# IanMadlenya/pyconsensus

Hardware: AMD Instinct MI355X
Metric: oracle rounds/sec (batched 50x20, 1 GPU) (higher is better)
Workload: dtype f64; 1 GPU; C3: 65536 independent 50x20 oracle rounds per GPU per step (one wavefront per round), inputs resident in HBM, every output of the result dict written (original and filled included); rounds_per_gpu=65536, reporters=50, events=20, parallelism=rounds sharded across 1 GPU(s), no collective

## Files before the change

pyconsensus_amd/csrc/pcx_api.cpp:

```cpp
#include <hip/hip_runtime.h>

#include <algorithm>
#include <atomic>
#include <cstdio>
#include <cstdlib>
#include <new>
#include <string>
#include <thread>
#include <vector>

#include "../../include/pcx.h"
#include "pcx_host.h"
#include "pcx_internal.h"
#include "pcx_seqsum.h"
#include "pcx_sync.h"

namespace pcx {
namespace host __attribute__((visibility("hidden"))) {
thread_local std::string g_err;

int fail(int code, const std::string& msg) {
    g_err = msg;
    return code;
}

int hip_fail(hipError_t e, const char* what) {
    return fail(PCX_EHIP, std::string(what) + ": " + hipGetErrorString(e));
}

void stamps_begin(pcx::BatchArgs& a, hipStream_t stream) {
    const char* env = getenv("PCX_STAMPS");
    if (!env || env[0] != '1' || a.B <= 0) return;
    const size_t bytes = (size_t)a.B * 32 * sizeof(long long);
    long long* d = nullptr;
    if (hipMalloc(&d, bytes) != hipSuccess) return;
    (void)hipMemsetAsync(d, 0, bytes, stream);
    a.stamps = d;
}

std::vector<long long> stamps_end(pcx::BatchArgs& a, hipStream_t stream) {
    std::vector<long long> h(a.stamps ? a.B * 32 : 0);
    if (!a.stamps) return h;
    (void)hipMemcpyAsync(h.data(), a.stamps, h.size() * sizeof(long long), hipMemcpyDeviceToHost, stream);
    (void)hipStreamSynchronize(stream);
    (void)hipFree(a.stamps);
    a.stamps = nullptr;
    return h;
}

int medium_scratch_reserve(pcx_ctx* ctx, size_t need) {
    if (ctx->mscr_bytes >= need) return PCX_OK;
    if (ctx->mscr) (void)hipFree(ctx->mscr);
    ctx->mscr = nullptr;
    ctx->mscr_bytes = 0;
    const hipError_t e = hipMalloc(&ctx->mscr, need);
    if (e != hipSuccess) return hip_fail(e, "hipMalloc(medium scratch)");
    ctx->mscr_bytes = need;
    return PCX_OK;
}
}
}
using namespace pcx::host;

extern "C" {

int pcx_abi_version(void) { return PCX_ABI_VERSION; }

const char* pcx_last_error(void) { return g_err.c_str(); }

namespace {
pcx_ctx* new_ctx(int device_id, const char* who) {
    int n = 0;
    hipError_t e = hipGetDeviceCount(&n);
    if (e != hipSuccess || device_id < 0 || device_id >= n) {
        g_err = std::string(who) + ": no HIP device " + std::to_string(device_id);
        return nullptr;
    }
    pcx_ctx* c = new (std::nothrow) pcx_ctx;
    if (!c) {
        g_err = std::string(who) + ": out of host memory";
        return nullptr;
    }
    c->device = device_id;
    return c;
}

pcx_ctx* with_comm(pcx_ctx* c, pcx::Comm* comm, const std::string& err) {
    if (!c) return nullptr;
    if (!comm) {
        g_err = err.empty() ? "communicator setup failed" : err;
        delete c;
        return nullptr;
    }
    c->comm = comm;
    return c;
}
}

pcx_ctx* pcx_create(int device_id) { return new_ctx(device_id, "pcx_create"); }

int pcx_comm_unique_id(pcx_comm_id* out) {
    if (!out) return fail(PCX_EINVAL, "pcx_comm_unique_id: null argument");
    std::string err;
    const int rc = pcx::comm_rccl_unique_id(out, err);
    return rc ? fail(rc, err) : PCX_OK;
}

pcx_ctx* pcx_create_rank(int device_id, int world, int rank, const pcx_comm_id* id) {
    if (!id || world < 1 || rank < 0 || rank >= world) {
        g_err = "pcx_create_rank: bad id / world / rank";
        return nullptr;
    }
    pcx_ctx* c = new_ctx(device_id, "pcx_create_rank");
    if (!c) return nullptr;
    std::string err;
    return with_comm(c, pcx::comm_rccl(device_id, world, rank, id, err), err);
}

pcx_group* pcx_group_create(int world) {
    pcx_group* g = pcx::group_create(world);
    if (!g) g_err = "pcx_group_create: world must be >= 1";
    return g;
}

void pcx_group_destroy(pcx_group* g) { pcx::group_destroy(g); }

pcx_ctx* pcx_create_grouped(int device_id, pcx_group* g, int rank) {
    pcx_ctx* c = new_ctx(device_id, "pcx_create_grouped");
    if (!c) return nullptr;
    std::string err;
    return with_comm(c, pcx::comm_group(g, rank, err), err);
}

pcx_ctx* pcx_create_custom(int device_id, int world, int rank, const pcx_comm_ops* ops) {
    pcx_ctx* c = new_ctx(device_id, "pcx_create_custom");
    if (!c) return nullptr;
    std::string err;
    return with_comm(c, pcx::comm_custom(world, rank, ops, err), err);
}

pcx_ctx* pcx_create_devices(int n_devices, const int* device_ids) {
    if (n_devices < 1 || !device_ids) {
        g_err = "pcx_create_devices: need n_devices >= 1 and device_ids";
        return nullptr;
    }
    pcx_ctx* c = new_ctx(device_ids[0], "pcx_create_devices");
    if (!c) return nullptr;
    for (int k = 1; k < n_devices; k++) {
        pcx_ctx* probe = new_ctx(device_ids[k], "pcx_create_devices");
        if (!probe) {
            delete c;
            return nullptr;
        }
        delete probe;
    }
    bool distinct = true;
    for (int a = 0; a < n_devices; a++)
        for (int b = a + 1; b < n_devices; b++) distinct = distinct && device_ids[a] != device_ids[b];
    std::string err;
    std::vector<pcx::Comm*> comms;
    if (distinct) {
        const int rc = pcx::comm_rccl_all(n_devices, device_ids, comms, err);
        if (rc) {
            g_err = "pcx_create_devices: " + err;
            delete c;
            return nullptr;
        }
    } else {
        c->group = pcx::group_create(n_devices);
        for (int k = 0; k < n_devices && c->group; k++) comms.push_back(pcx::comm_group(c->group, k, err));
    }
    for (int k = 0; k < n_devices; k++) {
        pcx_ctx* s = (k < (int)comms.size() && comms[k]) ? new (std::nothrow) pcx_ctx : nullptr;
        if (s) {
            s->device = device_ids[k];
            s->comm = comms[k];
        } else if (k < (int)comms.size()) {
            delete comms[k];
        }
        c->sub.push_back(s);
    }
    for (pcx_ctx* s : c->sub)
        if (!s) {
            g_err = "pcx_create_devices: communicator setup failed" + (err.empty() ? std::string() : ": " + err);
            pcx_destroy(c);
            return nullptr;
        }
    return c;
}

int pcx_ctx_world(const pcx_ctx* ctx) {
    if (ctx && !ctx->sub.empty()) return (int)ctx->sub.size();
    return ctx && ctx->comm ? ctx->comm->world : 1;
}
int pcx_ctx_rank(const pcx_ctx* ctx) { return ctx && ctx->comm ? ctx->comm->rank : 0; }

int pcx_ctx_usable(const pcx_ctx* ctx) {
    if (!ctx) return 0;
    if (ctx->comm && ctx->comm->aborted) return 0;
    for (const pcx_ctx* s : ctx->sub)
        if (s->comm && s->comm->aborted) return 0;
    return 1;
}

int pcx_release_workspace(pcx_ctx* ctx) {
    if (!ctx) return fail(PCX_EINVAL, "pcx_release_workspace: null context");
    for (pcx_ctx* s : ctx->sub) pcx_release_workspace(s);
    pcx::rounds_free(ctx);
    (void)hipSetDevice(ctx->device);
    pcx::workspace_free(ctx);
    pcx::io_bufs_free(ctx);
    pcx::sim_free(ctx);
    pcx::ragged_free(ctx);
    return PCX_OK;
}

}
namespace pcx {
void ctx_host_free(pcx_ctx* c) {
    if (c->mscr) (void)hipFree(c->mscr);
    c->mscr = nullptr;
    c->mscr_bytes = 0;
    if (c->pinned) (void)hipHostFree(c->pinned);
    c->pinned = nullptr;
    c->pinned_bytes = 0;
    if (c->sel_pin) (void)hipHostFree(c->sel_pin);
    c->sel_pin = nullptr;
    if (c->pin_small) (void)hipHostFree(c->pin_small);
    c->pin_small = nullptr;
    c->pin_small_bytes = 0;
    for (hipEvent_t& ev : c->sel_ev) {
        if (ev) (void)hipEventDestroy(ev);
        ev = nullptr;
    }
    if (c->side_stream) (void)hipStreamDestroy(c->side_stream);
    c->side_stream = nullptr;
    io_bufs_free(c);
}
void sim_free(pcx_ctx* c) {
    if (c->sim_buf) (void)hipFree(c->sim_buf);
    c->sim_buf = nullptr;
    c->sim_bytes = 0;
}
void ragged_free(pcx_ctx* c) {
    for (auto& s : c->rag) {
        if (s.copy_ev) (void)hipEventSynchronize(s.copy_ev);
        if (s.kern_ev) (void)hipEventSynchronize(s.kern_ev);
        if (s.pin) (void)hipHostFree(s.pin);
        if (s.dev) (void)hipFree(s.dev);
        if (s.copy_ev) (void)hipEventDestroy(s.copy_ev);
        if (s.kern_ev) (void)hipEventDestroy(s.kern_ev);
        s = pcx_ctx::RaggedSlot();
    }
}
void io_bufs_free(pcx_ctx* c) {
    for (auto& b : c->io_bufs)
        if (b.first) (void)hipFree(b.first);
    c->io_bufs.clear();
}
}
extern "C" {

void pcx_destroy(pcx_ctx* ctx) {
    if (!ctx) return;
    for (pcx_ctx* s : ctx->sub) pcx_destroy(s);
    if (ctx->group) pcx::group_destroy(ctx->group);
    pcx::rounds_free(ctx);
    (void)hipSetDevice(ctx->device);
    pcx::ctx_host_free(ctx);
    pcx::workspace_free(ctx);
    pcx::sim_free(ctx);
    pcx::ragged_free(ctx);
    delete ctx->comm;
    delete ctx;
}

int pcx_set_stream(pcx_ctx* ctx, void* s) {
    if (!ctx) return fail(PCX_EINVAL, "pcx_set_stream: null context");
    ctx->stream = reinterpret_cast<hipStream_t>(s);
    return PCX_OK;
}

int pcx_synchronize(pcx_ctx* ctx) {
    if (!ctx) return fail(PCX_EINVAL, "pcx_synchronize: null context");
    hipError_t e = hipSetDevice(ctx->device);
    if (e == hipSuccess) e = hipStreamSynchronize(ctx->stream);
    return e == hipSuccess ? PCX_OK : hip_fail(e, "pcx_synchronize");
}

static int batched_route(int64_t N, int64_t E, int alg, int k) {
    if (N < 1 || N > 0x7fffffff || E < 1 || E > 65536 || alg < PCX_ALG_PCA || alg > PCX_ALG_CLUSTERFECK) return -1;
    const bool large = N > 64 || E > 32;
    if (alg == PCX_ALG_KMEANS && (k < 1 || k > (large ? 1024 : 8) || k > N)) return -1;
    if (!large) return PCX_ROUTE_WAVE;
    return pcx::medium_fits((int)N, (int)E, alg, k) ? PCX_ROUTE_WORKGROUP : PCX_ROUTE_SCHEDULER;
}

int pcx_batched_route(int n_reporters, int n_events, int algorithm, int kmeans_k) {
    return batched_route(n_reporters, n_events, algorithm, kmeans_k);
}

static void print_wave_stamps(const std::vector<long long>& h, int64_t B) {
    static const int order[] = {0, 1, 2, 13, 14, 3, 4, 5, 6, 7, 8, 15, 16, 9, 10, 11, 12};
    const int no = (int)(sizeof(order) / sizeof(order[0]));
    double acc[32] = {0};
    for (int64_t b = 0; b < B; b++)
        for (int k = 1; k < no; k++) {
            const long long t1 = h[b * 32 + order[k]], t0 = h[b * 32 + order[k - 1]];
            if (t1 && t0) acc[order[k]] += (double)(t1 - t0);
        }
    fprintf(stderr, "PCX_STAMPS mean cycles per phase:");
    for (int k = 1; k < no; k++) fprintf(stderr, " %d:%.0f", order[k], acc[order[k]] / (double)B);
    double sort = 0, walk = 0, fast = 0, slow = 0;
    for (int64_t b = 0; b < B; b++) {
        sort += (double)h[b * 32 + 20];
        walk += (double)h[b * 32 + 21];
        fast += (double)h[b * 32 + 22];
        slow += (double)h[b * 32 + 23];
    }
    double iscr = 0, isort = 0;
    for (int64_t b = 0; b < B; b++) {
        iscr += (double)h[b * 32 + 24];
        isort += (double)h[b * 32 + 25];
    }
    fprintf(stderr, " median_sort:%.0f median_walk:%.0f outcome_shortcut:%.4f outcome_sorted:%.4f", sort / (double)B,
            walk / (double)B, fast / (double)B, slow / (double)B);
    fprintf(stderr, " interp_screened:%.4f interp_sorted:%.4f\n", iscr / (double)B, isort / (double)B);
}

static void print_medium_stamps(const std::vector<long long>& h, int64_t B) {
    double acc[16] = {0};
    for (int64_t b = 0; b < B; b++)
        for (int k = 1, prev = 0; k < 16; k++) {
            const long long t1 = h[b * 32 + k], t0 = h[b * 32 + prev];
            if (t1 && t0) {
                acc[k] += (double)(t1 - t0);
                prev = k;
            }
        }
    fprintf(stderr, "PCX_STAMPS medium mean cycles per phase:");
    for (int k = 1; k < 16; k++) fprintf(stderr, " %d:%.0f", k, acc[k] / (double)B);
    double mp[3] = {0, 0, 0};
    for (int64_t b = 0; b < B; b++)
        for (int k = 0; k < 3; k++) mp[k] += (double)h[b * 32 + 20 + k];
    fprintf(stderr, " wave0 medians total:%.0f rank:%.0f walk:%.0f", mp[0] / (double)B, mp[1] / (double)B,
            mp[2] / (double)B);
    double sub[4] = {0, 0, 0, 0};
    for (int64_t b = 0; b < B; b++)
        for (int k = 0; k < 4; k++) {
            const long long t1 = h[b * 32 + 24 + k], t0 = h[b * 32 + (k ? 23 + k : 8)];
            if (t1 && t0) sub[k] += (double)(t1 - t0);
        }
    fprintf(stderr, " nc: minmax+norm:%.0f n12:%.0f dots:%.0f ranks:%.0f", sub[0] / (double)B, sub[1] / (double)B,
            sub[2] / (double)B, sub[3] / (double)B);
    double pw[2] = {0, 0};
    for (int64_t b = 0; b < B; b++) {
        const long long* hb = &h[b * 32];
        if (hb[28] && hb[6]) pw[0] += (double)(hb[28] - hb[6]);
        if (hb[29] && hb[28]) pw[1] += (double)(hb[29] - hb[28]);
    }
    fprintf(stderr, " pi: presq:%.0f steps:%.0f\n", pw[0] / (double)B, pw[1] / (double)B);
}

static int run_workgroup_route(pcx_ctx* ctx, pcx::BatchArgs& a) {
    const int64_t chunk = pcx::medium_chunk(a, MEDIUM_SCRATCH_CAP);
    if (const int rc = medium_scratch_reserve(ctx, pcx::medium_scratch_per_round(a) * (size_t)chunk)) return rc;
    hipError_t e = hipSuccess;
    double* Fscr = (double*)ctx->mscr;
    double* Cscr = Fscr + (a.filled ? 0 : (size_t)chunk * a.N * a.E);
    double* Xscr = Cscr + (size_t)chunk * a.E * a.E;
    stamps_begin(a, ctx->stream);
    for (int64_t b0 = 0; b0 < a.B && e == hipSuccess; b0 += chunk)
        e = pcx::launch_medium(a, b0, std::min<int64_t>(chunk, a.B - b0), Fscr, Cscr, Xscr, ctx->stream);
    if (a.stamps) print_medium_stamps(stamps_end(a, ctx->stream), a.B);
    return e == hipSuccess ? PCX_OK : hip_fail(e, "medium_round_kernel launch");
}

int pcx_consensus_batched_f64(pcx_ctx* ctx, const pcx_batch* in, pcx_batch_result* out) {
    if (!ctx || !in || !out) return fail(PCX_EINVAL, "pcx_consensus_batched_f64: null argument");
    if (in->n_rounds < 0 || in->n_rounds > 0x7fffffff)
        return fail(PCX_EINVAL, "batched: n_rounds must be in [0, 2^31)");
    if (in->n_reporters < 1 || in->n_reporters > 0x7fffffff)
        return fail(PCX_EINVAL, "batched: n_reporters must be in [1, 2^31)");
    if (in->n_events < 1 || in->n_events > 65536) return fail(PCX_EINVAL, "batched: n_events must be in [1, 65536]");
    const bool large = in->n_reporters > 64 || in->n_events > 32;
    const char* own = nullptr;
    if (in->algorithm < PCX_ALG_PCA || in->algorithm > PCX_ALG_CLUSTERFECK)
        own = "algorithm must be an enum pcx_algorithm value (0..7)";
    else if (in->algorithm == PCX_ALG_KMEANS &&
             (!in->kmeans_init || in->kmeans_k < 1 || in->kmeans_k > (large ? 1024 : 8) ||
              in->kmeans_k > in->n_reporters || in->kmeans_restarts < 1))
        own = "k-means needs kmeans_init and 1 <= kmeans_k <= min(N, 8; 1024 above 64 x 32), restarts >= 1";
    else if (in->algorithm == PCX_ALG_BIG_FIVE && (in->max_components < 1 || in->max_components > in->n_events))
        own = "big-five needs 1 <= max_components <= n_events";
    if (const int rc = check_options("batched", in, own)) return rc;
    hipError_t e = hipSetDevice(ctx->device);
    if (e != hipSuccess) return hip_fail(e, "hipSetDevice");
    pcx::BatchArgs a = shared_args(in, out);
    a.B = in->n_rounds;
    a.N = (int)in->n_reporters;
    a.E = (int)in->n_events;
    a.ES = a.E | 1;
    a.bounds_shared = in->bounds_shared;
    a.kmeans_k = in->kmeans_k;
    a.kmeans_restarts = in->kmeans_restarts;
    a.kmeans_init = in->kmeans_init;
    const int route = batched_route(in->n_reporters, in->n_events, in->algorithm, in->kmeans_k);
    if (route < 0) return fail(PCX_EINVAL, "batched: invalid shape or algorithm");
    if (route == PCX_ROUTE_WORKGROUP && !getenv("PCX_NO_MEDIUM")) return run_workgroup_route(ctx, a);
    if (route != PCX_ROUTE_WAVE) {
        std::string err;
        const int rc = pcx::run_rounds(ctx, in, out, err);
        return rc ? fail(rc, "pcx_consensus_batched_f64: " + err) : PCX_OK;
    }
    stamps_begin(a, ctx->stream);
    e = pcx::launch_batched(a, ctx->stream);
    if (a.stamps) print_wave_stamps(stamps_end(a, ctx->stream), a.B);
    return e == hipSuccess ? PCX_OK : hip_fail(e, "batched_round_kernel launch");
}

namespace {
int run_devices(pcx_ctx* ctx, const pcx_problem* p, pcx_result* r, int entry, const double* scores, int rank_rule,
                double* nc, std::string& err) {
    const int n = (int)ctx->sub.size();
    const int64_t N = p->n_rows, E = p->n_events;
    if (p->mem_kind != PCX_MEM_HOST) {
        err = "a multi-device context takes the matrix in host memory (PCX_MEM_HOST)";
        return PCX_EINVAL;
    }
    if (p->n_total != N || p->row_offset != 0) {
        err = "a multi-device context takes the whole matrix (n_total == n_rows, row_offset 0)";
        return PCX_EINVAL;
    }
    if (N < n || E < 1 || !p->reports) {
        err = "bad shape (fewer rows than devices) or missing reports";
        return PCX_EINVAL;
    }
    if (const int rc = pcx::check_problem(p, n, entry, err)) return rc;
    std::vector<pcx_problem> ps(n, *p);
    std::vector<pcx_result> rs(n);
    std::vector<std::string> errs(n);
    std::vector<int> rcs;
    const int64_t base = N / n, rem = N % n;
    auto at = [](double* a, int64_t off) { return a ? a + off : nullptr; };
    for (int k = 0; k < n; k++) {
        const int64_t off = k * base + (k < rem ? k : rem), cnt = base + (k < rem ? 1 : 0);
        pcx_problem& q = ps[k];
        q.n_rows = cnt;
        q.n_total = N;
        q.row_offset = off;
        q.reports = p->reports + off * E;
        q.aux_scores = p->aux_scores ? p->aux_scores + off : nullptr;
        pcx_result& o = rs[k];
        o = pcx_result{};
        o.old_rep = at(r->old_rep, off);
        o.this_rep = at(r->this_rep, off);
        o.smooth_rep = at(r->smooth_rep, off);
        o.scores = at(r->scores, off);
        o.na_row = at(r->na_row, off);
        o.participation_rows = at(r->participation_rows, off);
        o.relative_part = at(r->relative_part, off);
        o.reporter_bonus = at(r->reporter_bonus, off);
        o.original = at(r->original, off * E);
        o.filled = at(r->filled, off * E);
        if (k == 0) {
            o.adj_first_loadings = r->adj_first_loadings;
            o.outcomes_raw = r->outcomes_raw;
            o.outcomes_adjusted = r->outcomes_adjusted;
            o.outcomes_final = r->outcomes_final;
            o.certainty = r->certainty;
            o.consensus_reward = r->consensus_reward;
            o.nas_filled = r->nas_filled;
            o.participation_columns = r->participation_columns;
            o.author_bonus = r->author_bonus;
            o.weighted_mean = r->weighted_mean;
            o.covariance = r->covariance;
        }
    }
    pcx::run_workers(
        n,
        [&](int k) {
            const int64_t off = ps[k].row_offset;
            return pcx::run_matrix(ctx->sub[k], &ps[k], &rs[k], entry, scores ? scores + off : nullptr, rank_rule,
                                   nc ? nc + off : nullptr, errs[k]);
        },
        [&](int k) {
            if (ctx->group) pcx::group_abort(ctx->group);
            for (pcx_ctx* o : ctx->sub)
                if (o->comm && o != ctx->sub[k]) o->comm->abort();
        },
        rcs);
    if (ctx->group) pcx::group_reset(ctx->group);
    int first = -1;
    for (int k = 0; k < n && first < 0; k++)
        if (rcs[k] && errs[k].find("exchange aborted") == std::string::npos) first = k;
    for (int k = first < 0 ? 0 : first; k < n; k++)
        if (rcs[k]) {
            err = "device " + std::to_string(ctx->sub[k]->device) + " (rank " + std::to_string(k) + "): " + errs[k];
            return rcs[k];
        }
    double bytes = 0;
    for (int k = 0; k < n; k++) bytes += rs[k].comm_bytes;
    const pcx_result& z = rs[0];
    r->participation = z.participation;
    r->avg_certainty = z.avg_certainty;
    r->branch = z.branch;
    r->flags = z.flags;
    r->pi_iters = z.pi_iters;
    r->components = z.components;
    r->n_hard = z.n_hard;
    r->sel_passes = z.sel_passes;
    r->comm_bytes = bytes;
    r->grid_events = z.grid_events;
    r->mixed_int8 = z.mixed_int8;
    return 0;
}

int run(pcx_ctx* ctx, const pcx_problem* p, pcx_result* r, int entry, const double* scores, int rank_rule, double* nc,
        const char* who) {
    if (!ctx || !p || !r) return fail(PCX_EINVAL, std::string(who) + ": null argument");
    std::string err;
    if (!ctx->sub.empty()) {
        const int rc = run_devices(ctx, p, r, entry, scores, rank_rule, nc, err);
        return rc ? fail(rc, std::string(who) + ": " + err) : PCX_OK;
    }
    const int rc = pcx::run_matrix(ctx, p, r, entry, scores, rank_rule, nc, err);
    return rc ? fail(rc, std::string(who) + ": " + err) : PCX_OK;
}
}

int pcx_consensus_f64(pcx_ctx* ctx, const pcx_problem* p, pcx_result* r) {
    return run(ctx, p, r, 0, nullptr, 0, nullptr, "pcx_consensus_f64");
}

int pcx_interpolate_f64(pcx_ctx* ctx, const pcx_problem* p, pcx_result* r) {
    return run(ctx, p, r, 1, nullptr, 0, nullptr, "pcx_interpolate_f64");
}

int pcx_wpca_f64(pcx_ctx* ctx, const pcx_problem* p, pcx_result* r) {
    return run(ctx, p, r, 2, nullptr, 0, nullptr, "pcx_wpca_f64");
}

int pcx_lie_detector_f64(pcx_ctx* ctx, const pcx_problem* p, pcx_result* r) {
    return run(ctx, p, r, 3, nullptr, 0, nullptr, "pcx_lie_detector_f64");
}

int pcx_nonconformity_f64(pcx_ctx* ctx, const pcx_problem* p, const double* scores, int rank_rule, double* nc,
                          pcx_result* r) {
    if (!scores || !nc) return fail(PCX_EINVAL, "pcx_nonconformity_f64: scores and nc are required");
    return run(ctx, p, r, 4, scores, rank_rule, nc, "pcx_nonconformity_f64");
}

int pcx_profile_enable(pcx_ctx* ctx, int on) {
    if (!ctx) return fail(PCX_EINVAL, "pcx_profile_enable: null context");
    for (pcx_ctx* s : ctx->sub) s->profile = on ? 1 : 0;
    ctx->profile = on ? 1 : 0;
    return PCX_OK;
}

int pcx_profile_read(pcx_ctx* ctx, double* ms) {
    if (!ctx || !ms) return fail(PCX_EINVAL, "pcx_profile_read: null argument");
    const pcx_ctx* src = ctx->sub.empty() ? ctx : ctx->sub[0];
    for (int k = 0; k < PCX_NSTAGES; k++) ms[k] = src->stage_ms[k];
    return PCX_OK;
}

const char* pcx_stage_name(int k) { return pcx::stage_name(k); }

int pcx_ctx_progress(const pcx_ctx* ctx, int* stage, int* host_waiting) {
    if (!ctx || !stage || !host_waiting) return fail(PCX_EINVAL, "pcx_ctx_progress: null argument");
    const pcx_ctx* src = ctx->sub.empty() ? ctx : ctx->sub[0];
    *stage = src->progress_stage.load(std::memory_order_relaxed);
    *host_waiting = src->progress_wait.load(std::memory_order_relaxed);
    return PCX_OK;
}

double pcx_seqsum_const(double c, int64_t k) { return pcx::seqsum_const(c, k); }

int64_t pcx_seqsum_first_above(double c, double t, int64_t kmax) { return pcx::seqsum_first_above(c, t, kmax); }
int pcx_mixed_digits(void) { return PCX_NDIG; }
int pcx_rccl_version(int* runtime, int* compiled) { return pcx::rccl_version(runtime, compiled); }
int pcx_selftest_abort_once(int users, int aborters, int iters) {
    return pcx::selftest_abort_once(users, aborters, iters, 0);
}
int pcx_selftest_abort_slow_holder(int users, int aborters) {
    return pcx::selftest_abort_once(users, aborters, 1, 1);
}
int pcx_selftest_group_abort(int world, int steps, int fail_rank, int fail_step) {
    return pcx::selftest_group_abort(world, steps, fail_rank, fail_step);
}
int pcx_selftest_rounds_sched(int workers, int64_t rounds, int enomem_worker, int64_t fail_round) {
    return pcx::selftest_rounds_sched(workers, rounds, enomem_worker, fail_round);
}
int pcx_selftest_chunked_copy(int64_t bytes, int64_t chunk, int slots, int threads, int64_t fail_chunk) {
    return pcx::selftest_chunked_copy(bytes, chunk, slots, threads, fail_chunk);
}
int64_t pcx_medium_lds_bytes(int n_reporters, int n_events, int algorithm) {
    if (!pcx::medium_fits(n_reporters, n_events, algorithm, 1)) return 0;
    return (int64_t)pcx::medium_lds_bytes(n_reporters, n_events, algorithm);
}

int64_t pcx_batched_lds_bytes(int n_reporters, int n_events, int algorithm) {
    if (n_reporters < 1 || n_reporters > 64 || n_events < 1 || n_events > 32) return -1;
    return (int64_t)pcx::batched_lds_bytes(n_reporters, n_events, algorithm);
}
int pcx_test_inject_enomem(pcx_ctx* ctx, int worker) {
    if (!ctx) return fail(PCX_EINVAL, "pcx_test_inject_enomem: null context");
    ctx->test_enomem_worker = worker;
    return PCX_OK;
}

}
```

pyconsensus_amd/csrc/pcx_batched_round.inc:

```
#if PCX_ROUND_RAGGED >= 2
#define PCX_ROUND_CELL0 rcell
#define PCX_ROUND_ROW0 rrow
#define PCX_ROUND_EV0 rev
#define PCX_ROUND_B rround
template <int NT, int ET, bool CLUS, bool PK>
#if PCX_ROUND_RAGGED == 3
__global__ void __launch_bounds__(64, 3) ragged_kmeans_round_kernel(BatchArgs ka, const MediumDesc* __restrict__ rag,
                                                                    const RoundParams* __restrict__ ptab,
                                                                    const KmeansEntry* __restrict__ ktab) {
#else
__global__ void __launch_bounds__(64, 3) ragged_params_round_kernel(BatchArgs ka, const MediumDesc* __restrict__ rag,
                                                                    const RoundParams* __restrict__ ptab) {
#endif
    static_assert(NT == 0 && ET == 0, "a ragged launch has no compiled shape");
    extern __shared__ __attribute__((aligned(16))) double smem[];
    const MediumDesc* const rd = rag + blockIdx.x;
    const int N = __builtin_amdgcn_readfirstlane(rd->N), E = __builtin_amdgcn_readfirstlane(rd->E), ES = E | 1;
    const int64_t rcell = uniform64(rd->cell), rrow = uniform64(rd->row), rev = uniform64(rd->ev);
    const int64_t rround = __builtin_amdgcn_readfirstlane(rd->round);
    const RoundParams* const rp = ptab + __builtin_amdgcn_readfirstlane(rd->param);
    BatchArgs a = ka;
    a.algorithm = __builtin_amdgcn_readfirstlane(rp->algorithm);
    a.max_components = __builtin_amdgcn_readfirstlane(rp->max_components);
    a.catch_tol = uniform_f64(rp->catch_tol);
    a.alpha = uniform_f64(rp->alpha);
    a.variance_threshold = uniform_f64(rp->variance_threshold);
    a.hierarchy_threshold = uniform_f64(rp->hierarchy_threshold);
    a.cluster_threshold = uniform_f64(rp->cluster_threshold);
#if PCX_ROUND_RAGGED == 3
    const KmeansEntry* const ke = ktab + rround;
    a.kmeans_k = __builtin_amdgcn_readfirstlane(ke->k);
    a.kmeans_init = ka.kmeans_init + uniform64(ke->offset);
#endif
#elif PCX_ROUND_RAGGED
#define PCX_ROUND_CELL0 rcell
#define PCX_ROUND_ROW0 rrow
#define PCX_ROUND_EV0 rev
#define PCX_ROUND_B blockIdx.x
template <int NT, int ET, bool CLUS, bool PK>
__global__ void __launch_bounds__(64, 3) ragged_round_kernel(BatchArgs a, const RaggedDesc* __restrict__ rag) {
    static_assert(NT == 0 && ET == 0, "a ragged launch has no compiled shape");
    extern __shared__ __attribute__((aligned(16))) double smem[];
    const RaggedDesc* const rd = rag + blockIdx.x;
    const int N = __builtin_amdgcn_readfirstlane(rd->N), E = __builtin_amdgcn_readfirstlane(rd->E), ES = E | 1;
    const int64_t rcell = uniform64(rd->cell), rrow = uniform64(rd->row), rev = uniform64(rd->ev);
#else
#define PCX_ROUND_CELL0 (b * (int64_t)N * E)
#define PCX_ROUND_ROW0 (b * N)
#define PCX_ROUND_EV0 (b * E)
#define PCX_ROUND_B blockIdx.x
template <int NT, int ET, bool CLUS, bool PK>
__global__ void __launch_bounds__(64, (NT > 0 && PK) ? PACKED_WAVES : 3) batched_round_kernel(BatchArgs a) {
    extern __shared__ __attribute__((aligned(16))) double smem[];
    const int N = NT > 0 ? NT : a.N, E = ET > 0 ? ET : a.E, ES = ET > 0 ? compiled_es(ET) : a.ES;
#endif
    const int l = lane_id();
    const int64_t b = PCX_ROUND_B;
    constexpr int NRM = NT > 0 ? NT : 64;
    Smem S = carve(smem, N, E, ES, NRM, PK);
    const bool row = l < N, col = l < E;
    const int64_t bo = a.bounds_shared ? 0 : PCX_ROUND_EV0;
    const bool has_bounds = a.scaled != nullptr;
    auto pw_rows = [&](double v) { return wave_pw_sum_prefix<NT>(v, N); };
    auto pw_cols = [&](double v) { return wave_pw_sum_prefix<ET>(v, E); };
    constexpr int CR = live_rows(ET);

    typedef const __attribute__((address_space(4))) BatchArgs* KernArgs;
    auto out_args = [&]() -> KernArgs {
        uint64_t p = (uint64_t)__builtin_amdgcn_kernarg_segment_ptr();
        asm volatile("" : "+s"(p));
        return (KernArgs)p;
    };

    long long mprof[3] = {0, 0, 0};
    STAMP(0);
    const double* Rg = a.reports + PCX_ROUND_CELL0;
    bool scj = false;
    double loj = 0.0, hij = 0.0;
    if (col && has_bounds) {
        scj = a.scaled[bo + l] != 0;
        loj = a.lo[bo + l];
        hij = a.hi[bo + l];
    }
    double raw = row && a.reputation ? a.reputation[PCX_ROUND_ROW0 + l] : 0.0;
    if constexpr (NT > 0 && ET > 0 && (NT * ET) % 2 == 0) {
        constexpr int TOT2 = NT * ET / 2, NV = (TOT2 + W - 1) / W;
        double2 v[NV];
#pragma unroll
        for (int q = 0; q < NV; q++)
            if (l + W * q < TOT2) v[q] = reinterpret_cast<const double2*>(Rg)[l + W * q];
#pragma unroll
        for (int q = 0; q < NV; q++) {
            const int idx = 2 * (l + W * q);
            if (idx < NT * ET) {
                const int i0 = idx / ET, j0 = idx - i0 * ET;
                const int i1 = (idx + 1) / ET, j1 = idx + 1 - i1 * ET;
                S.F[i0 * ES + j0] = v[q].x;
                S.F[i1 * ES + j1] = v[q].y;
            }
        }
    } else {
        for (int idx = l; idx < N * E; idx += W) {
            const int i = idx / E, j = idx - i * E;
            S.F[i * ES + j] = Rg[idx];
        }
    }
    const uint64_t scaled_mask = ballot(col && scj);

    double rep;
    if (a.reputation) {
        const double tot = pw_rows(raw);
        rep = raw / tot;
    } else {
        rep = 1.0 / (double)N;
    }
    const double tok = trunc(rep * 1e6);
    if (row) S.rep[l] = rep;
    const double denom = tree_sum(row ? tok : 0.0) - 1.0;
    wsync();

    STAMP(1);
    uint32_t nacnt = 0;
    double xnext = row ? S.F[l * ES] : 1.0;
    uint32_t nanb = 0, zerob = 0;
    int zcol = 0;
#pragma unroll(ET > 0 ? ET : 1)
    for (int j = 0; j < E; j++) {
        const bool sc = (scaled_mask >> j) & 1;
        double x = xnext;
        if (j + 1 < E) xnext = row ? S.F[l * ES + j + 1] : 1.0;
        if (sc) {
            const double lo = bcast(loj, j), hi = bcast(hij, j);
            if (row) {
                x = (x - lo) / (hi - lo);
                if (a.int_dtype) x = trunc(x);
                S.F[l * ES + j] = x;
            }
        }
        const bool xn = __builtin_isnan(x), xz = x == 0.0;
        nanb |= xn ? 1u << j : 0u;
        zerob |= xz ? 1u << j : 0u;
        const uint64_t zm = ballot(xz), mm = ballot(xn) | zm;
        zcol = l == j ? popc(zm) : zcol;
        if (l == 0) S.miss[j] = mm;
        asm volatile("" : "+v"(nanb), "+v"(zerob), "+v"(zcol));
    }
    nacnt = (uint32_t)__popc(zerob) | ((uint32_t)__popc(nanb) << 8) | ((uint32_t)zcol << 16);
    wsync();
    if (double* const og = out_args()->original) round_to_global(og + PCX_ROUND_CELL0, S.F, N, E, ES, NT, ET);

    STAMP(2);
    uint64_t miss_j = 0;
    if (col) miss_j = S.miss[l];
    {
        constexpr int NR = NT > 0 ? NT : 64;
        double tot = 0.0, sp = 0.0, sa = 0.0;
#pragma unroll 10
        for (int i = 0; i < NR; i++) {
            if (i < N) {
                const bool miss = (miss_j >> i) & 1;
                const double re = miss ? 0.0 : S.rep[i];
                const double f = miss ? 0.0 : S.F[i * ES + (col ? l : 0)];
                tot = tot + re;
                sp = fma(re, f, sp);
                sa = fma(fabs(re), fabs(f), sa);
            }
        }
        const double t_lo = 1.5 - a.catch_tol, t_hi = 1.5 + a.catch_tol;
        const double accf = sp / tot, margin = 1e-12 * (sa / tot);
        const bool binary_fill = col && miss_j && !scj;
        const bool fast = tot > 0.0 && __builtin_isfinite(accf) && __builtin_isfinite(margin) &&
                          fabs(accf - t_lo) > margin && fabs(accf - t_hi) > margin;
        double acc = accf;
        if (ballot(binary_fill && !fast)) {
            double ex = 0.0;
#pragma unroll
            for (int i = 0; i < NR; i++) {
                if (i < N) {
                    const double t = (S.rep[i] / tot) * S.F[i * ES + (col ? l : 0)];
                    ex = ((miss_j >> i) & 1) ? ex : ex + t;
                }
            }
            if (!fast) acc = ex;
        }
        if (binary_fill) {
            double g = catch_(acc, a.catch_tol);
            if (a.int_dtype) g = trunc(g);
            S.guess[l] = g;
        }
        if (col && miss_j) S.tot[l] = tot;
    }
    wsync();
    STAMP(13);
    {
        uint64_t todo = ballot(col && scj && miss_j != 0);
        auto pair_of = [&](int j, double& x, double& w, bool& present) {
            const uint64_t mj = S.miss[j];
            present = row && !((mj >> l) & 1);
            const double tot = S.tot[j];
            x = row ? S.F[l * ES + j] : 0.0;
            w = present ? S.rep[l] / tot : 0.0;
        };
        auto finish = [&](int j, double g) {
            if (a.int_dtype) g = trunc(g);
            if (l == 0) S.guess[j] = g;
        };
        constexpr int NRS = NT > 0 ? NT : 64, KP = (NRS + 3) & ~3;
        const uint64_t all_j = todo;
        if (todo && a.reputation && !ballot(row && !(rep >= 0.0))) {
            uint32_t* const kx = reinterpret_cast<uint32_t*>(S.M);
            float* const wf = reinterpret_cast<float*>(S.M) + KP;
            if (l < KP) wf[l] = row ? (float)rep : 0.f;
            for (uint64_t t = todo; t; t &= t - 1) {
                const int j = __builtin_ctzll(t);
                const uint64_t mj = S.miss[j];
                const bool present = row && !((mj >> l) & 1);
                const double x0 = row ? S.F[l * ES + j] : 0.0;
                double g;
                if (wave_wmedian_screen<NRS>(x0, rep, present, S.tot[j], N, kx, wf, g)) {
                    finish(j, g);
                    todo &= ~(1ull << j);
                }
            }
            wsync();
        }
        if (a.stamps && l == 0) {
            a.stamps[b * 32 + 24] = popc(all_j) - popc(todo);
            a.stamps[b * 32 + 25] = popc(todo);
        }
        while (todo) {
            const int j = __builtin_ctzll(todo);
            todo &= todo - 1;
            double x0, w0;
            bool p0;
            pair_of(j, x0, w0, p0);
            finish(j, wave_wmedian_rank<(NT > 0 ? NT : 64)>(x0, w0, p0, N, S.M, a.stamps ? mprof : nullptr));
            wsync();
        }
    }
    wsync();
    STAMP(14);
    if (row) {
        uint64_t mn = S.miss[0];
        double gn = S.guess[0];
        for (int j = 0; j < E; j++) {
            const uint64_t mj = mn;
            const double g = gn;
            if (j + 1 < E) {
                mn = S.miss[j + 1];
                gn = S.guess[j + 1];
            }
            if ((mj >> l) & 1) S.F[l * ES + j] = g;
        }
    }
    wsync();
    if (double* const fg = out_args()->filled) round_to_global(fg + PCX_ROUND_CELL0, S.F, N, E, ES, NT, ET);

    STAMP(3);
    double oldj = col ? ob_vecmat(S.rep, S.F + l, ES, N, E, l) : 0.0;

    double sc_i = 0.0, nc_i = 0.0, ld_j = 0.0;
    int branch = 5, flags = 0, iters = 0, comps = -1;
    const int alg = a.algorithm;
    const bool clus = CLUS && alg >= 5;
    const double rep_sum = pw_rows(rep);
    if (alg == 0 || alg == 2 || alg == 3 || clus) {
        const double den = rep_sum;
        double muj = 0.0;
        if (E == 1) {
            const double p = row ? S.F[l * ES] * rep : 0.0;
            const double acc = pw_rows(p);
            muj = acc / den;
        } else if (col) {
            double acc = S.F[l] * S.rep[0];
            for (int i = 1; i < N; i++) acc = acc + S.F[i * ES + l] * S.rep[i];
            muj = acc / den;
        }
        if constexpr (!PK) {
            wsync();
            if (col) S.mu[l] = muj;
            wsync();
        }

        STAMP(4);
        bool nonzero = false, finite = true;
        {
            constexpr int NR = NT > 0 ? NT : 64;
            const int ml = l & 15, kq = l >> 4;
            const bool two = E > 16;
            const double m0 = __shfl(muj, ml), m1 = __shfl(muj, 16 + ml);
            const double mu0 = ml < E ? m0 : 0.0, mu1 = 16 + ml < E ? m1 : 0.0;
            d4v c00 = {0, 0, 0, 0}, c10 = {0, 0, 0, 0}, c11 = {0, 0, 0, 0};
#pragma unroll
            for (int i0 = 0; i0 < NR; i0 += 4) {
                if (i0 < N) {
                    const int i = i0 + kq;
                    const bool ok = i < N;
                    const double tk = ok ? trunc(S.rep[i] * 1e6) : 0.0;
                    const bool v0 = ok && ml < E, v1 = ok && 16 + ml < E;
                    const double d0 = v0 ? S.F[i * ES + ml] - mu0 : 0.0;
                    const double d1 = v1 ? S.F[i * ES + 16 + ml] - mu1 : 0.0;
                    const double a0 = v0 ? d0 * tk : 0.0, a1 = v1 ? d1 * tk : 0.0;
                    c00 = mfma_f64(a0, d0, c00);
                    if (two) {
                        c10 = mfma_f64(a1, d0, c10);
                        c11 = mfma_f64(a1, d1, c11);
                    }
                }
            }
            auto put = [&](int j, int k, double acc) {
                const double c = acc / denom;
                S.C[sym_at<PK>(j, k, ES)] = c;
                if (!PK) {
                    S.M[sym_at<PK>(j, k, ES)] = c;
                    S.C[k * ES + j] = c;
                    S.M[k * ES + j] = c;
                }
                nonzero |= c != 0.0;
                finite &= __builtin_isfinite(c) != 0;
            };
            if constexpr (PK) wsync();
#pragma unroll
            for (int r = 0; r < 4; r++) {
                const int j0 = kq + 4 * r, j1 = 16 + kq + 4 * r, k0 = ml, k1 = 16 + ml;
                if (j0 < E && k0 <= j0) put(j0, k0, c00[r]);
                if (j1 < E && k0 < E) put(j1, k0, c10[r]);
                if (j1 < E && k1 <= j1) put(j1, k1, c11[r]);
            }
        }
        const bool any_nz = ballot(nonzero) != 0;
        const bool all_fin = ballot(!finite) == 0;
        wsync();

        STAMP(5);
        double xv = 0.0;
        if (!all_fin) {
            xv = col ? 1.0 : 0.0;
            flags |= 2;
        } else if (!any_nz) {
            xv = l == 0 ? 1.0 : 0.0;
            flags |= 1;
        } else {
            const double dg = col ? S.C[sym_at<PK>(l, l, ES)] : -__builtin_inf();
            const double dgmax = wave_max<CR>(dg);
            const int kd = __builtin_ctzll(ballot(col && dg == dgmax));
            double x0 = col ? S.C[sym_at<PK>(l, kd, ES)] : 0.0;
            const double n0 = sqrt(tree_sum<CR>(x0 * x0));
            xv = col ? x0 / n0 : 0.0;
            constexpr int NS = !PK ? 1 : ET > 0 ? (ET + 3) / 4 : EMAX / 4;
            SymOps<NS> mreg, creg;
            if constexpr (PK) {
                load_sym_ops<NS>(S.C, E, mreg);
                creg = mreg;
            }
            auto square = [&](bool in_loop) {
                if constexpr (PK) {
                    if (in_loop) load_sym_ops<NS>(S.C, E, mreg);
                    square_scaled_reg<NS>(mreg, E);
                    if (in_loop) store_sym_ops<NS>(S.C, E, mreg);
                } else {
                    square_scaled<PK>(S.M, ES, E);
                }
            };
            int sqn = 0;
            for (; sqn < PI_PRESQUARE; sqn++) square(false);
            if constexpr (PK) store_sym_ops<NS>(S.C, E, mreg);
            int it = 0, since = 0;
            for (;;) {
                const double y = matvec_unit<PK, CR>(PK ? S.C : S.M, ES, xv, E);
                const bool moved = ballot(col && fabs(y - xv) > PI_TOL) != 0;
                xv = y;
                it++;
                since++;
                if (!moved) break;
                if (it >= PI_MAXIT) {
                    flags |= 4;
                    break;
                }
                if (since >= PI_SQUARE_EVERY && sqn < PI_MAX_SQUARINGS) {
                    square(true);
                    sqn++;
                    since = 0;
                }
            }
            if constexpr (PK) store_sym_ops<NS>(S.C, E, creg);
            for (int p = 0; p < PI_POLISH; p++) xv = matvec_unit<PK, CR>(S.C, ES, xv, E);
            const uint64_t nzm = ballot(col && xv != 0.0);
            if (nzm) {
                const double xf = bcast(xv, __builtin_ctzll(nzm));
                const bool neg = popc(nzm) == 1 ? xf < 0.0 : xf > 0.0;
                if (neg) xv = -xv;
            }
            iters = it + PI_POLISH + sqn;
        }
        const double nv = sqrt(pw_cols(xv * xv));
        ld_j = col ? xv / nv : 0.0;
        wsync();
        if (clus) {
        } else if (alg == 0) {
            const int r = row ? l : 0;
            double acc = 0.0;
            for (int j = 0; j < E; j++) acc = fma(S.F[r * ES + j] - lane_value(muj, j), lane_value(ld_j, j), acc);
            if (row) sc_i = acc;
        } else if (flags & 2) {
            sc_i = __builtin_nan("");
        } else if constexpr (!PK) {
            const double trace = pw_cols(col ? S.C[l * ES + l] : 0.0);
            wsync();
            for (int o = l; o < E * E; o += W) {
                const int j = o / E, k = o - j * E;
                S.M[j * ES + k] = S.C[j * ES + k];
            }
            wsync();
            jacobi_eig_wave(S.M, S.C, ES, E, S.x, S.ld);
            const double sig = col ? fabs(S.M[l * ES + l]) : 0.0;
            if (col) S.nv1[l] = sig;
            wsync();
            if (col) {
                int rk = 0;
                for (int k = 0; k < E; k++) rk += (S.nv1[k] > sig) | ((S.nv1[k] == sig) & (k < l));
                S.nv2[rk] = (double)l;
            }
            wsync();
#if PCX_ROUND_RAGGED
            const int kmax = alg == 2 && a.max_components < E ? a.max_components : E;
#else
            const int kmax = alg == 2 ? a.max_components : E;
#endif
            double net = 0.0, ve = 0.0;
            int used = kmax;
            for (int c = 0; c < kmax; c++) {
                const int idx = (int)S.nv2[c];
                const double sg = S.nv1[idx];
                const double fl = S.C[idx] < 0.0 ? -1.0 : 1.0;
                if (row) {
                    double d = 0.0;
                    for (int j = 0; j < E; j++) d = fma(S.F[l * ES + j] - S.mu[j], fl * S.C[j * ES + idx], d);
                    net = net + sg * d;
                }
                if (alg == 3) {
                    ve = ve + sg / trace;
                    if (ve >= a.variance_threshold) {
                        used = c + 1;
                        break;
                    }
                }
            }
            comps = alg == 3 ? used : -1;
            sc_i = net;
            wsync();
        }
    } else if (alg == 4) {
        sc_i = row ? a.aux_scores[PCX_ROUND_ROW0 + l] : 0.0;
    }
    STAMP(6);
    if constexpr (CLUS) {
        if (clus) {
            double* X = smem + smem_doubles(N, E, ES, NRM, PK);
            if (alg == 6)
                nc_i = hier_nc(S.F, S.mu, ES, N, E, a.hierarchy_threshold, reinterpret_cast<uint64_t*>(X));
#if !PCX_ROUND_RAGGED
            else if (alg == 5)
                nc_i = kmeans_nc(a, b, S.F, S.mu, ES, N, E, X);
#elif PCX_ROUND_RAGGED == 3
            else if (alg == 5)
                nc_i = kmeans_nc(a, 0, S.F, S.mu, ES, N, E, X);
#endif
            else
                nc_i = feck_nc(a, S.F, ES, N, E, rep, X);
            wsync();
        }
    }
    if (alg != 1 && !clus) {
        const bool any_nan = ballot(row && __builtin_isnan(sc_i)) != 0;
        double mn = wave_max(row ? -sc_i : -__builtin_inf());
        mn = -mn;
        double mx = wave_max(row ? sc_i : -__builtin_inf());
        if (any_nan) {
            mn = __builtin_nan("");
            mx = __builtin_nan("");
        }
        const double set1 = sc_i + fabs(mn);
        const double set2 = sc_i - mx;
        double a1 = fabs(set1), a2 = fabs(set2);
        double S1 = pw_rows(a1);
        if (S1 == 0) {
            a1 += 1.0;
            S1 = pw_rows(a1);
        }
        double S2 = pw_rows(a2);
        if (S2 == 0) {
            a2 += 1.0;
            S2 = pw_rows(a2);
        }
        if (row) {
            S.n1[l] = a1 / S1;
            S.n2[l] = a2 / S2;
        }
        if (col) S.old[l] = oldj;
        wsync();
        double d1 = 0.0, d2 = 0.0;
        {
            const int jc = l & 31;
            double d = 0.0;
            if (jc < E) d = ob_vecmat(l < 32 ? S.n1 : S.n2, S.F + jc, ES, N, E, jc);
            const uint64_t du = (uint64_t)__double_as_longlong(d);
            const int up = ((l + 32) & 63) << 2;
            const uint32_t ulo = (uint32_t)__builtin_amdgcn_ds_bpermute(up, (int)(uint32_t)du);
            const uint32_t uhi = (uint32_t)__builtin_amdgcn_ds_bpermute(up, (int)(uint32_t)(du >> 32));
            if (col) {
                d1 = d;
                d2 = __longlong_as_double((long long)(((uint64_t)uhi << 32) | ulo));
            }
        }
        if (col) {
            const double t = 0.01 * oldj;
            S.nv1[l] = d1 + t;
            S.nv2[l] = d2 + t;
        }
        wsync();
        double ref = 0.0;
        if (alg == 0) {
            double r0, r1, r2;
            if (3 * E <= W) {
                rank_avg3(S.old, S.nv1, S.nv2, E, r0, r1, r2);
            } else {
                r0 = rank_avg(S.old, E);
                r1 = rank_avg(S.nv1, E);
                r2 = rank_avg(S.nv2, E);
            }
            const double e1 = fabs(r1 - r0), e2 = fabs(r2 - r0);
            ref = pw_cols(e1) - pw_cols(e2);
        }
        bool pick1;
        if (ref == 0) {
            const double q1 = d1 - oldj, q2 = d2 - oldj;
            const double ref2 = pw_cols(q1 * q1) - pw_cols(q2 * q2);
            pick1 = ref2 <= 0;
            branch = pick1 ? 3 : 4;
        } else {
            pick1 = ref < 0;
            branch = pick1 ? 1 : 2;
        }
        nc_i = pick1 ? set1 : set2;
    }

    STAMP(7);
    const double meanrep = rep_sum / (double)N;
    double u = fabs(nc_i * (rep / meanrep));
    double Su = pw_rows(u);
    const bool rep_masked = alg == 0 && __builtin_isnan(Su);
    if (Su == 0) {
        u += 1.0;
        Su = pw_rows(u);
    }
    const double this_i = u / Su;
    const double smooth_i = a.alpha * this_i + (1.0 - a.alpha) * rep;
    wsync();
    if (row) S.smooth[l] = smooth_i;
    wsync();

    STAMP(8);
    double lo2 = NT > 0 ? 0.0 : loj, hi2 = NT > 0 ? 0.0 : hij;
    if constexpr (NT > 0) {
        if (col && scj) {
            lo2 = a.lo[bo + l];
            hi2 = a.hi[bo + l];
        }
    }
    double rawj = col ? ob_vecmat(S.smooth, S.F + l, ES, N, E, l) : 0.0;
    STAMP(15);
    if (scaled_mask) {
        const double Wt = tree_sum(row ? smooth_i : 0.0);
        const double mid = 0.5 * Wt, slack = 0x1p-45 * Wt;
        const double Mg = 0x1p-44 * Wt + slack + DBL_EPS;
        const bool wok = Mg < __builtin_inf() && !ballot(row && !(smooth_i >= 0.0 && smooth_i < mid - slack)) &&
                         ballot(row && smooth_i > 0.0) != 0;
        uint64_t slow = 0;
        for (uint64_t todo = scaled_mask; todo; todo &= todo - 1) {
            const int j = __builtin_ctzll(todo);
            const double x0 = row ? S.F[l * ES + j] : 0.0;
            const uint64_t mj = (uint64_t)uniform64((int64_t)S.miss[j]);
            bool decided = false;
            if (wok && mj) {
                const double g = bcast(x0, __builtin_ctzll(mj));
                if (g != 0.0 && fabs(g) < 0x1p1023 && !ballot(row && x0 != x0)) {
                    const double below = tree_sum(row && x0 < g ? smooth_i : 0.0);
                    const double group = tree_sum(row && x0 == g ? smooth_i : 0.0);
                    decided = below <= mid - Mg && below + group > mid + Mg;
                    if (decided && l == j) rawj = g;
                }
            }
            if (!decided) slow |= 1ull << j;
        }
        if (a.stamps && l == 0) {
            a.stamps[b * 32 + 22] = popc(scaled_mask) - popc(slow);
            a.stamps[b * 32 + 23] = popc(slow);
        }
        while (slow) {
            const int j = __builtin_ctzll(slow);
            slow &= slow - 1;
            const double x0 = row ? S.F[l * ES + j] : 0.0;
            const double m = wave_wmedian_rank<(NT > 0 ? NT : 64)>(x0, smooth_i, row, N, S.M, a.stamps ? mprof : nullptr);
            if (l == j) rawj = m;
            wsync();
        }
    }
    STAMP(16);
    double adjj = 0.0, finj = 0.0;
    if (col) {
        if (scj) {
            adjj = rawj;
            finj = adjj * (hi2 - lo2);
            finj = finj + lo2;
        } else {
            adjj = catch_(rawj, a.catch_tol);
            finj = adjj;
        }
        S.adj[l] = adjj;
    }
    wsync();

    STAMP(9);
    double certj = 0.0;
    {
        uint64_t* hitm = reinterpret_cast<uint64_t*>(S.M);
        double fn = row ? S.F[l * ES] : 0.0, an = S.adj[0];
        for (int j = 0; j < E; j++) {
            const double f = fn, av = an;
            if (j + 1 < E) {
                fn = row ? S.F[l * ES + j + 1] : 0.0;
                an = S.adj[j + 1];
            }
            const uint64_t hm = ballot(row && f == av);
            if (l == 0) hitm[j] = hm;
        }
        wsync();
        const int NS = cert_stride(N, ES);
        double* comp = S.F;
        for (int j = 0; j < E; j++) {
            const uint64_t hm = hitm[j];
            if ((hm >> l) & 1) comp[j * NS + mbcnt64(hm)] = smooth_i;
        }
        wsync();
        if (col) {
            constexpr int TMAX = (NT > 0 ? NT : 64) / 8;
            const uint64_t hm = hitm[l];
            const int n = popc(hm), T = n >> 3;
            const double* c = comp + l * NS;
            double res = 0.0;
            if (T) {
                double r[8];
#pragma unroll
                for (int k = 0; k < 8; k++) r[k] = c[k];
#pragma unroll
                for (int t = 1; t < TMAX; t++)
                    if (t < T) {
#pragma unroll
                        for (int k = 0; k < 8; k++) r[k] = r[k] + c[8 * t + k];
                    }
                res = ((r[0] + r[1]) + (r[2] + r[3])) + ((r[4] + r[5]) + (r[6] + r[7]));
            }
            for (int q = 8 * T; q < n; q++) res = res + c[q];
            certj = n ? res : (a.algorithm == 0 ? __builtin_nan("") : 0.0);
        }
    }
    double ac = fabs(certj);
    double Sc = pw_cols(ac);
    if (Sc == 0) {
        ac += 1.0;
        Sc = pw_cols(ac);
    }
    const double reward = ac / Sc;
    const double avg_cert = pw_cols(certj) / (double)E;

    STAMP(10);
    double pcj = 0.0, nzj = 0.0;
    const bool smooth_finite = !ballot(row && !__builtin_isfinite(smooth_i));
    if (col) {
        const uint64_t nam = S.miss[l];
        double s = 0.0, c = 0.0;
        auto step = [&](double x, double y) {
            const double p = x * y;
            const double pe = fma(x, y, -p);
            const double t = s + p;
            const double z = t - s;
            const double se = (s - (t - z)) + (p - z);
            s = t;
            c = c + (pe + se);
        };
        if (smooth_finite) {
            for (uint64_t mm = nam; mm; mm &= mm - 1) step(S.smooth[__builtin_ctzll(mm)], 1.0);
        } else {
            for (int i = 0; i < N; i++) step(S.smooth[i], ((nam >> i) & 1) ? 1.0 : 0.0);
        }
        pcj = 1.0 - (s + c);
        nzj = (double)((nacnt >> 16) & 0xffu);
    }
    double narow = 0.0;
    int nnan = 0;
    if (row) {
        narow = (double)(nacnt & 0xffu);
        nnan = (int)((nacnt >> 8) & 0xffu);
    }
    const bool rowmasked = row && nnan == E;
    const double pr = 1.0 - narow / (double)E;
    const double pna = 1.0 - pw_cols(pcj) / (double)E;
    double ar = rowmasked ? 0.0 : fabs(pr);
    double Sr = pw_rows(ar);
    if (Sr == 0) {
        ar = rowmasked ? 0.0 : fabs(pr) + 1.0;
        Sr = pw_rows(ar);
    }
    const double rel = rowmasked ? fabs(pr) : ar / Sr;
    double apc = fabs(pcj);
    double Spc = pw_cols(apc);
    if (Spc == 0) {
        apc += 1.0;
        Spc = pw_cols(apc);
    }
    const double relc = apc / Spc;

    STAMP(11);
    const auto oa = out_args();
    if (row) {
        const int64_t o = PCX_ROUND_ROW0 + l;
        if (oa->old_rep) oa->old_rep[o] = rep;
        if (oa->this_rep) oa->this_rep[o] = this_i;
        if (oa->smooth_rep) oa->smooth_rep[o] = smooth_i;
        if (oa->scores) oa->scores[o] = sc_i;
        if (oa->na_row) oa->na_row[o] = narow;
        if (oa->participation_rows) oa->participation_rows[o] = pr;
        if (oa->relative_part) oa->relative_part[o] = rel;
        if (oa->reporter_bonus) oa->reporter_bonus[o] = (rowmasked || rep_masked) ? rel : rel * pna + smooth_i * (1.0 - pna);
    }
    if (col) {
        const int64_t o = PCX_ROUND_EV0 + l;
        if (oa->adj_first_loadings) oa->adj_first_loadings[o] = ld_j;
        if (oa->outcomes_raw) oa->outcomes_raw[o] = rawj;
        if (oa->outcomes_adjusted) oa->outcomes_adjusted[o] = adjj;
        if (oa->outcomes_final) oa->outcomes_final[o] = finj;
        if (oa->certainty) oa->certainty[o] = certj;
        if (oa->consensus_reward) oa->consensus_reward[o] = reward;
        if (oa->nas_filled) oa->nas_filled[o] = nzj;
        if (oa->participation_columns) oa->participation_columns[o] = rep_masked ? 1.0 : pcj;
        if (oa->author_bonus) oa->author_bonus[o] = rep_masked ? 1.0 : relc * pna + reward * (1.0 - pna);
    }
    if (l == 0) {
        if (oa->participation) oa->participation[b] = 1.0 - pna;
        if (oa->avg_certainty) oa->avg_certainty[b] = avg_cert;
        if (oa->branch) oa->branch[b] = branch;
        if (oa->flags) oa->flags[b] = flags;
        if (oa->pi_iters) oa->pi_iters[b] = iters;
        if (oa->components) oa->components[b] = comps;
    }
    STAMP(12);
    if (a.stamps && threadIdx.x == 0) {
        a.stamps[b * 32 + 20] = mprof[0];
        a.stamps[b * 32 + 21] = mprof[1];
    }
}
#undef PCX_ROUND_CELL0
#undef PCX_ROUND_ROW0
#undef PCX_ROUND_EV0
#undef PCX_ROUND_B
```

Before: 64.41 million rounds/s.

## Split binary-fill column sums across three lane groups with exact replay fallback

When reputations are nonnegative and 3*E fits in a wavefront, the per-column weighted sums over reporters are split across three lane groups, each covering every third reporter, and combined with lane permutes. This cuts the serial reporter loop roughly threefold for 20-event rounds. The exact sequential total and the slow binary-fill path are moved into a replay stage that runs only when the fast margin test fails or the scaled median needs a bit-exact total. It adds permute traffic and more code, plus new stamp counters for the replay rate.

```diff
diff --git a/pyconsensus_amd/csrc/pcx_api.cpp b/pyconsensus_amd/csrc/pcx_api.cpp
--- a/pyconsensus_amd/csrc/pcx_api.cpp
+++ b/pyconsensus_amd/csrc/pcx_api.cpp
@@ -325,7 +325,13 @@
     }
     fprintf(stderr, " median_sort:%.0f median_walk:%.0f outcome_shortcut:%.4f outcome_sorted:%.4f", sort / (double)B,
             walk / (double)B, fast / (double)B, slow / (double)B);
-    fprintf(stderr, " interp_screened:%.4f interp_sorted:%.4f\n", iscr / (double)B, isort / (double)B);
+    double grep = 0, gtot = 0;
+    for (int64_t b = 0; b < B; b++) {
+        grep += (double)h[b * 32 + 26];
+        gtot += (double)h[b * 32 + 27];
+    }
+    fprintf(stderr, " interp_screened:%.4f interp_sorted:%.4f", iscr / (double)B, isort / (double)B);
+    fprintf(stderr, " guess_replayed:%.4f replay_rounds:%.4f\n", grep / (double)B, gtot / (double)B);
 }
 
 static void print_medium_stamps(const std::vector<long long>& h, int64_t B) {
diff --git a/pyconsensus_amd/csrc/pcx_batched_round.inc b/pyconsensus_amd/csrc/pcx_batched_round.inc
--- a/pyconsensus_amd/csrc/pcx_batched_round.inc
+++ b/pyconsensus_amd/csrc/pcx_batched_round.inc
@@ -152,41 +152,75 @@
     STAMP(2);
     uint64_t miss_j = 0;
     if (col) miss_j = S.miss[l];
+    const bool nonneg = !ballot(row && !(rep >= 0.0));
+    const bool binary_fill = col && miss_j && !scj;
+    bool tot_exact;
+    uint64_t need_bin = 0;
     {
-        constexpr int NR = NT > 0 ? NT : 64;
+        constexpr bool SPLITC = NT > 0 && ET > 0 && 3 * ET <= W;
+        const bool split = SPLITC ? nonneg : (nonneg && 3 * E <= W);
+        const bool sums = SPLITC ? nonneg : true;
+        tot_exact = SPLITC ? false : !split;
         double tot = 0.0, sp = 0.0, sa = 0.0;
-#pragma unroll 10
-        for (int i = 0; i < NR; i++) {
-            if (i < N) {
-                const bool miss = (miss_j >> i) & 1;
+        const int g = split ? (l >= E) + (l >= 2 * E) : 0;
+        const bool live = l < (split ? 3 * E : E);
+        const int c = live ? l - g * E : 0;
+        uint64_t m = ~0ull;
+        if (sums) {
+            const uint64_t past = N < 64 ? ~0ull << N : 0ull;
+            const uint64_t mc = split ? S.miss[c] : miss_j;
+            m = live ? ((mc | past) >> g) | ~(~0ull >> g) : ~0ull;
+        }
+        if constexpr (SPLITC) {
+            if (split) {
+                constexpr int TS = (NT + 2) / 3;
+                const double* const Fp = S.F + g * ES + c;
+                const double* const rp = S.rep + g;
+                const uint32_t mlo = (uint32_t)m, mhi = (uint32_t)(m >> 32);
+#pragma unroll
+                for (int t = 0; t < TS; t++) {
+                    const bool miss = ((3 * t < 32 ? mlo : mhi) & (1u << ((3 * t) & 31))) != 0;
+                    const double r0 = rp[3 * t];
+                    const uint64_t fu = (uint64_t)__double_as_longlong(Fp[3 * t * ES]);
+                    const uint32_t fh = miss ? 0u : (uint32_t)(fu >> 32);
+                    const double re = miss ? 0.0 : r0;
+                    const double f = __longlong_as_double((long long)(((uint64_t)fh << 32) | (uint32_t)fu));
+                    tot = tot + re;
+                    sp = fma(re, f, sp);
+                    sa = fma(re, fabs(f), sa);
+                }
+            }
+        } else {
+            const int G = split ? 3 : 1;
+            const double* const Fc = S.F + c;
+            for (int k = 0; k < N; k += G) {
+                const bool miss = (m >> k) & 1;
+                const int i = g + k;
                 const double re = miss ? 0.0 : S.rep[i];
-                const double f = miss ? 0.0 : S.F[i * ES + (col ? l : 0)];
+                const double f = miss ? 0.0 : Fc[i * ES];
                 tot = tot + re;
                 sp = fma(re, f, sp);
                 sa = fma(fabs(re), fabs(f), sa);
             }
         }
+        if (split) {
+            const int l1 = (l + E) & (W - 1), l2 = (l + 2 * E) & (W - 1);
+            const double t1 = bpermute_d(l1, tot), t2 = bpermute_d(l2, tot);
+            const double p1 = bpermute_d(l1, sp), p2 = bpermute_d(l2, sp);
+            const double a1 = bpermute_d(l1, sa), a2 = bpermute_d(l2, sa);
+            tot = (tot + t1) + t2;
+            sp = (sp + p1) + p2;
+            sa = (sa + a1) + a2;
+        }
         const double t_lo = 1.5 - a.catch_tol, t_hi = 1.5 + a.catch_tol;
         const double accf = sp / tot, margin = 1e-12 * (sa / tot);
-        const bool binary_fill = col && miss_j && !scj;
-        const bool fast = tot > 0.0 && __builtin_isfinite(accf) && __builtin_isfinite(margin) &&
+        const bool fast = sums && tot > 0.0 && __builtin_isfinite(accf) && __builtin_isfinite(margin) &&
                           fabs(accf - t_lo) > margin && fabs(accf - t_hi) > margin;
-        double acc = accf;
-        if (ballot(binary_fill && !fast)) {
-            double ex = 0.0;
-#pragma unroll
-            for (int i = 0; i < NR; i++) {
-                if (i < N) {
-                    const double t = (S.rep[i] / tot) * S.F[i * ES + (col ? l : 0)];
-                    ex = ((miss_j >> i) & 1) ? ex : ex + t;
-                }
-            }
-            if (!fast) acc = ex;
-        }
-        if (binary_fill) {
-            double g = catch_(acc, a.catch_tol);
-            if (a.int_dtype) g = trunc(g);
-            S.guess[l] = g;
+        need_bin = ballot(binary_fill && !fast);
+        if (binary_fill && fast) {
+            double gs = catch_(accf, a.catch_tol);
+            if (a.int_dtype) gs = trunc(gs);
+            S.guess[l] = gs;
         }
         if (col && miss_j) S.tot[l] = tot;
     }
@@ -207,7 +241,7 @@
         };
         constexpr int NRS = NT > 0 ? NT : 64, KP = (NRS + 3) & ~3;
         const uint64_t all_j = todo;
-        if (todo && a.reputation && !ballot(row && !(rep >= 0.0))) {
+        if (todo && a.reputation && nonneg) {
             uint32_t* const kx = reinterpret_cast<uint32_t*>(S.M);
             float* const wf = reinterpret_cast<float*>(S.M) + KP;
             if (l < KP) wf[l] = row ? (float)rep : 0.f;
@@ -227,6 +261,41 @@
         if (a.stamps && l == 0) {
             a.stamps[b * 32 + 24] = popc(all_j) - popc(todo);
             a.stamps[b * 32 + 25] = popc(todo);
+        }
+        const bool replay = need_bin || (todo && !tot_exact);
+        if (a.stamps && l == 0) {
+            a.stamps[b * 32 + 26] = popc(need_bin);
+            a.stamps[b * 32 + 27] = replay;
+        }
+        if (replay) {
+            constexpr int NR = NT > 0 ? NT : 64;
+            const double* const Fc = S.F + (col ? l : 0);
+            double tot = 0.0;
+#pragma unroll 10
+            for (int i = 0; i < NR; i++) {
+                if (i < N) {
+                    const bool miss = (miss_j >> i) & 1;
+                    const double re = miss ? 0.0 : S.rep[i];
+                    tot = tot + re;
+                }
+            }
+            if (need_bin) {
+                double ex = 0.0;
+#pragma unroll 10
+                for (int i = 0; i < NR; i++) {
+                    if (i < N) {
+                        const double t = (S.rep[i] / tot) * Fc[i * ES];
+                        ex = ((miss_j >> i) & 1) ? ex : ex + t;
+                    }
+                }
+                if ((need_bin >> l) & 1) {
+                    double gs = catch_(ex, a.catch_tol);
+                    if (a.int_dtype) gs = trunc(gs);
+                    S.guess[l] = gs;
+                }
+            }
+            if (col && miss_j) S.tot[l] = tot;
+            wsync();
         }
         while (todo) {
             const int j = __builtin_ctzll(todo);
```

Result: faster. 66.23 million rounds/s (median of 6 runs) (+2.8%).
